# jrcalgo/RelayRL-prototype

Hardware: AMD Instinct MI355X
Metric: env steps/sec (whole node) + wall-clock to return threshold, CartPole REINFORCE (higher is better)
Workload: dtype fp32; 1 GPU; global_batch=2097152, seq_len=64, parallelism=dp1, envs_per_gpu=32768, train_vf_iters=80, hyperparams=reference defaults (gamma .98, lam .97, pi_lr 3e-4, vf_lr 1e-3)

## Files before the change

### csrc/kernels/value_grad.hip

```cpp
#include <type_traits>

#include "api.h"
#include "common.h"
#include "grad_args.h"
#include "heads.h"

namespace rrl {

typedef __bf16 vbf16x8 __attribute__((ext_vector_type(8)));
typedef __bf16 vbf16x4 __attribute__((ext_vector_type(4)));
typedef short vs16x4 __attribute__((ext_vector_type(4)));

constexpr int kVgH = 128;
#ifndef VG_MT2
#define VG_MT2 1
#endif
constexpr int kVgLd = 144;
constexpr int kVgImg = 64 * kVgLd;
constexpr int vg_red_bytes(int NA) { return 8 * 64 * NA * 4; }
constexpr int vg_base_bytes(int DP, int NA) {
  return 6 * kVgImg * 2 + 2 * 64 * DP * 4 + (2 + NA) * 128 * 4 + 32 * 4 + kVgH * kVgLd * 2;
}
constexpr bool vg_red_in_image(int DP, int NA) { return vg_base_bytes(DP, NA) + vg_red_bytes(NA) > 160 * 1024; }
constexpr int vg_lds_bytes(int DP, int NA) {
// ... 161 lines not shown
  const vs16x4 hi = __builtin_amdgcn_ds_read_tr16_b64_v4i16((lds_v4*)(a0 + 4 * kVgLd));
  typedef short vs16x8 __attribute__((ext_vector_type(8)));
  const vs16x8 v = __builtin_shufflevector(lo, hi, 0, 1, 2, 3, 4, 5, 6, 7);
  return __builtin_bit_cast(vbf16x8, v);
}
RRL_DEV Split8 frag_tr(const uint16_t* img, int k0, int col0, int lane) {
  Split8 s;
  s.h = frag_tr1(img, k0, col0, lane);
  s.m = frag_tr1(img + kVgImg, k0, col0, lane);
  s.l = frag_tr1(img + 2 * kVgImg, k0, col0, lane);
  return s;
}

RRL_DEV void store_split(uint16_t* img, int row, int col, const floatx4 v) {
  vbf16x4 h, m, lo;
  split4(v, h, m, lo);
  uint16_t* a = img + img_off(row, col);
  *reinterpret_cast<vbf16x4*>(a) = h;
  *reinterpret_cast<vbf16x4*>(a + kVgImg) = m;
  *reinterpret_cast<vbf16x4*>(a + 2 * kVgImg) = lo;
}

struct Pieces {
  vbf16x4 h, m, l;
};
RRL_DEV void store_pieces(uint16_t* img, int row, int col, const Pieces& pc) {
  uint16_t* a = img + img_off(row, col);
  *reinterpret_cast<vbf16x4*>(a) = pc.h;
  *reinterpret_cast<vbf16x4*>(a + kVgImg) = pc.m;
  *reinterpret_cast<vbf16x4*>(a + 2 * kVgImg) = pc.l;
}

template <int CTRL>
RRL_DEV float dpp_f(float v) {
  return __int_as_float(__builtin_amdgcn_update_dpp(0, __float_as_int(v), CTRL, 0xf, 0xf, true));
}
constexpr int kDppXor8 = 0x128;
constexpr int kDppMirror8 = 0x141;
constexpr int kDppXor2 = 0x4e;
constexpr int kDppXor1 = 0xb1;

RRL_DEV float reduce_scatter16(const float (&v)[16], int j) {
  float u[8], w4[4], w2[2];
#pragma unroll
  for (int k = 0; k < 8; ++k) {
    const bool hi = j & 8;
    const float send = hi ? v[k] : v[k + 8], keep = hi ? v[k + 8] : v[k];
    u[k] = keep + dpp_f<kDppXor8>(send);
  }
#pragma unroll
  for (int k = 0; k < 4; ++k) {
    const bool hi = j & 4;
    const float send = hi ? u[k] : u[k + 4], keep = hi ? u[k + 4] : u[k];
    w4[k] = keep + dpp_f<kDppMirror8>(send);
  }
#pragma unroll
  for (int k = 0; k < 2; ++k) {
    const bool hi = j & 2;
    const float send = hi ? w4[k] : w4[k + 2], keep = hi ? w4[k + 2] : w4[k];
    w2[k] = keep + dpp_f<kDppXor2>(send);
  }
  const bool hi = j & 1;
  const float send = hi ? w2[0] : w2[1], keep = hi ? w2[1] : w2[0];
  return keep + dpp_f<kDppXor1>(send);
}

RRL_DEV float wave_sum_vl(float v) {
  v += dpp_f<kDppXor1>(v);
  v += dpp_f<kDppXor2>(v);
  v += dpp_f<kDppMirror8>(v);
  v += dpp_f<kDppXor8>(v);
  return group_sum_swap(v);
}

#define VG_STAMP(k)                                                                     \
  if (STAMP) {                                                                          \
    __builtin_amdgcn_sched_barrier(0);                                                  \
    unsigned long long t_;                                                              \
    asm volatile("s_memtime %0\n\ts_waitcnt lgkmcnt(0)" : "=s"(t_)::"memory");          \
    __builtin_amdgcn_sched_barrier(0);                                                  \
    if ((k) > 0) st_sum[(k) > 0 ? (k)-1 : 0] += t_ - st_prev;                           \
    st_prev = t_;                                                                       \
  }

constexpr int vg_prod_v(int DP) { return DP <= 4 ? 7 : 1; }

template <int DP, int HEAD, int NA, bool STAMP = false, int V = vg_prod_v(DP), bool FWD = false>
__global__ __launch_bounds__(512, 1) void value_grad_split_kernel(GradArgs p) {
  unsigned long long st_prev = 0, st_sum[12] = {0, 0, 0, 0, 0, 0, 0, 0, 0, 0, 0, 0};
  unsigned long long st_entry = 0;
  if (STAMP) asm volatile("s_memtime %0\n\ts_waitcnt lgkmcnt(0)" : "=s"(st_entry)::"memory");
  extern __shared__ __attribute__((aligned(16))) uint16_t vg_lds[];
  constexpr bool kValue = HEAD == HEAD_VALUE_MSE;
  constexpr bool kGauss = HEAD == HEAD_PG_GAUSS || HEAD == HEAD_PPO_GAUSS;
  constexpr bool kPPO = HEAD == HEAD_PPO_CAT || HEAD == HEAD_PPO_GAUSS;
  static_assert(!kValue || NA == 1, "the value head has one output");
  static_assert(!FWD || kValue, "the forward-only instance is the value head's");
  static_assert(NA >= 1 && NA <= 6, "NA <= 6 (LDS plan, two field groups)");
  static_assert(!vg_split_head(HEAD, NA) || (NA % 2 == 0 && NA <= 6),
                "the dout table is read in output pairs; head MFMA lanes g = 0, 1 hold outputs 0..7");
  constexpr bool kFactor = vg_factor(DP, HEAD, NA) && !FWD;
  constexpr bool kBin = kFactor && !kValue;
  constexpr bool kMaskB = kFactor && (V & 1);
  constexpr bool kInterleave = kMaskB && (V & 2);
  constexpr bool kPipe = kInterleave && !FWD && vg_pipe(DP, HEAD, V);
  constexpr int NF = NA + 2;
  constexpr int NG = (NF + 3) / 4;
  constexpr bool kRedImg = vg_red_in_image(DP, NA);
  constexpr bool kSplitHead = vg_split_head(HEAD, NA);
  uint16_t* h1img = vg_lds;
  uint16_t* dhimg = vg_lds + 3 * kVgImg;
  float* tail = reinterpret_cast<float*>(vg_lds + 6 * kVgImg);
  float* red = kRedImg ? reinterpret_cast<float*>(dhimg) : tail;
  float* xsb = kRedImg ? tail : tail + 8 * NA * 64;
  float* vecs = xsb + 2 * 64 * DP;
  uint16_t* w2lo = reinterpret_cast<uint16_t*>(vecs + (2 + NA) * kVgH + 32);
  uint32_t* mk = reinterpret_cast<uint32_t*>(w2lo + kVgH * kVgLd);
  const vbf16x8* mtab = reinterpret_cast<const vbf16x8*>(mk + 64 * 4);
  float* hbuf0 = kRedImg ? red + 8 * NA * 64
                         : reinterpret_cast<float*>(reinterpret_cast<char*>(mk) + vg_mask_bytes(DP, HEAD, NA));
  float* dtab = reinterpret_cast<float*>(
      reinterpret_cast<char*>(mk) + vg_mask_bytes(DP, HEAD, NA) +
      (kRedImg ? 0 : (vg_hbuf2(DP, HEAD, NA) ? 2 : 1) * vg_hbuf_bytes(HEAD, NA)));
  float* hacc = dtab + 64 * NA;
  float* xs3 = reinterpret_cast<float*>(reinterpret_cast<char*>(vg_lds) + vg_total_bytes(DP, HEAD, NA));
  uint16_t* mbt = reinterpret_cast<uint16_t*>(xs3 + 64 * DP) + 64 * (threadIdx.x >> 6);
  uint16_t* dpt = reinterpret_cast<uint16_t*>(xs3 + 64 * DP) + 8 * 64;
  if (kSplitHead && lane_id() < 2 * NA) hacc[(threadIdx.x >> 6) * 2 * NA + lane_id()] = 0.f;
  if (kMaskB) {
    for (int q = threadIdx.x; q < 256 * 4; q += blockDim.x) {
      const int i = q >> 2, e = 2 * (q & 3);
      mk[64 * 4 + q] = (((i >> e) & 1) ? 0x3F80u : 0u) | (((i >> (e + 1)) & 1) ? 0x3F800000u : 0u);
    }
  }
  int parity = 0;
  int xi = 0;
  constexpr int KS1 = DP / 4;
  const int l = lane_id();
  const int j = l & 15, g = l >> 4, w = threadIdx.x >> 6;
  const int D = p.D;
  const int Bv = p.nvalid ? min(*p.nvalid, p.B) : p.B;
  const int Bc = max(Bv, 1);
  const float invB = p.inv_B_dev ? *p.inv_B_dev : p.inv_B;
  const FlatOffsets o = flat_offsets(D, kVgH, NA);
  float adv_mean = 0.f, adv_rstd = 1.f;
  if (!kValue && p.adv_stats != nullptr) {
    const float n = fmaxf(p.adv_stats[2], 1.f);
    adv_mean = p.adv_stats[0] / n;
    const float var = fmaxf(p.adv_stats[1] / n - adv_mean * adv_mean, 0.f);
    adv_rstd = 1.f / (sqrtf(var) + 1e-8f);
  }
  const float* __restrict__ P = p.params;
  const int own = 16 * w;
  auto frag_slot = [&]() {
    int ll = l;
    asm volatile("" : "+v"(ll));
    return (ll & 32) + 8 * ((ll >> 2) & 3) + ((ll >> 2) & 4) + (ll & 3);
  };

  constexpr int NC = kGauss ? NA : 1;
  const int wu = __builtin_amdgcn_readfirstlane(w);
  auto dma = [&](const void* src, long n, long first, float* dst, int chunks, int w0) {
    for (int k = 0; k < chunks; ++k) {
      if (((k + w0) & 7) == wu) {
        const long e = min(first + 64L * k + l, n - 1);
        __builtin_amdgcn_global_load_lds(static_cast<const uint32_t*>(src) + e,
                                         (__attribute__((address_space(3))) void*)(dst + 64 * k), 4, 0, 0);
      }
    }
  };
  constexpr bool kDmaIn = !kValue;
  constexpr int XQ = (64 * DP + 511) / 512;
  float xr[kDmaIn ? 1 : XQ];
  float hin_r = 0.f;
  auto prefetch_x = [&](int b0, float* dst) {
    if (kDmaIn) {
      for (int k = wu; k < DP; k += 8) {
        const int q = 64 * k + l, row = q / DP, d = q % DP;
        const long e = (long)min(b0 + row, Bc - 1) * D + min(d, D - 1);
        __builtin_amdgcn_global_load_lds(static_cast<const uint32_t*>(static_cast<const void*>(p.X)) + e,
                                         (__attribute__((address_space(3))) void*)(dst + 64 * k), 4, 0, 0);
      }
    } else {
#pragma unroll
      for (int i = 0; i < (kDmaIn ? 1 : XQ); ++i) {
        const int q = min((int)threadIdx.x + 512 * i, 64 * DP - 1);
        const int rl = q / DP, d = q % DP, b = b0 + rl;
        xr[i] = p.X[(size_t)min(b, Bc - 1) * D + min(d, D - 1)];
      }
      if (!FWD) hin_r = p.ret[min(b0 + l, p.B - 1)];
    }
  };
  auto xbuf = [&](int i) { return i < 2 ? xsb + i * 64 * DP : xs3; };
  auto load_x = [&](int b0) {
    int tid = threadIdx.x;
    asm volatile("" : "+v"(tid));
#pragma unroll
    for (int i = 0; i < (kDmaIn ? 1 : XQ); ++i) {
      const int q = min(tid + 512 * i, 64 * DP - 1);
      const int rl = q / DP, d = q % DP, b = b0 + rl;
      xr[i] = p.X[(size_t)min(b, Bc - 1) * D + min(d, D - 1)];
    }
  };
  auto store_x = [&](int b0, float* dst) {
    int tid = threadIdx.x;
    asm volatile("" : "+v"(tid));
#pragma unroll
    for (int i = 0; i < (kDmaIn ? 1 : XQ); ++i) {
      const int q = tid + 512 * i;
      const int rl = q / DP, d = q % DP;
      if (q < 64 * DP) dst[q] = (b0 + rl < Bv && d < D) ? xr[i] : 0.f;
    }
  };
  constexpr bool kHb2 = kDmaIn && vg_hbuf2(DP, HEAD, NA);
  constexpr int HBF = vg_hbuf_bytes(HEAD, NA) / 4;
  auto dma_head = [&](int b0, float* hbuf) {
    if (kDmaIn) {
      dma(p.adv, p.B, b0, hbuf, 1, 3);
      if (p.logp_old) dma(p.logp_old, p.B, b0, hbuf + 64, 1, 4);
      if (kGauss) dma(p.actc, (long)p.B * NA, (long)b0 * NA, hbuf + 128, NA, 5);
      else dma(p.act, p.B, b0, hbuf + 128, 1, 5);
    }
  };
  auto vm_wait0 = []() { __builtin_amdgcn_s_waitcnt(0x0F70); };
  prefetch_x(blockIdx.x * 64, xsb);
  if (kHb2) dma_head(blockIdx.x * 64, hbuf0);

  constexpr int kW2Ld = kVgH + 4;
  static_assert(kVgH * kW2Ld * 4 <= 6 * kVgImg * 2, "staged W2 must fit in the activation images");
  float* w2s = reinterpret_cast<float*>(vg_lds);
  float* hsc = vecs + (2 + NA) * kVgH;
  float w1a[KS1];
#pragma unroll
  for (int s = 0; s < KS1; ++s) {
    const int k = 4 * s + g;
    w1a[s] = (k < D) ? P[o.w1 + (own + j) * D + k] : 0.f;
  }
  {
    const float* gw2 = P + o.w2;
    const bool al16 = (reinterpret_cast<uintptr_t>(gw2) & 15) == 0;
    floatx4 v[kVgH * kVgH / 4 / 512];
#pragma unroll
    for (int it = 0; it < kVgH * kVgH / 4 / 512; ++it) {
      const int q = (int)threadIdx.x + 512 * it;
      if (al16) {
        v[it] = *reinterpret_cast<const floatx4*>(gw2 + 4 * q);
      } else {
#pragma unroll
        for (int e = 0; e < 4; ++e) v[it][e] = gw2[4 * q + e];
      }
    }
    for (int q = threadIdx.x; q < (2 + NA) * kVgH; q += blockDim.x) {
      const int k = q >> 7, f = q & (kVgH - 1);
      vecs[q] = P[(k == 0 ? o.b1 : k == 1 ? o.b2 : o.w3 + (k - 2) * kVgH) + f];
    }
    if (threadIdx.x < NA) {
      const int a = threadIdx.x;
      const float lsa = kGauss ? P[o.log_std + a] : 0.f;
      hsc[a] = P[o.b3 + a];
      hsc[NA + a] = lsa;
      hsc[2 * NA + a] = __expf(-lsa);
    }
#pragma unroll
    for (int it = 0; it < kVgH * kVgH / 4 / 512; ++it) {
      const int q = (int)threadIdx.x + 512 * it;
      *reinterpret_cast<floatx4*>(w2s + (q >> 5) * kW2Ld + 4 * (q & 31)) = v[it];
      vbf16x4 h, m, lo;
      split4(v[it], h, m, lo);
      *reinterpret_cast<vbf16x4*>(w2lo + (q >> 5) * kVgLd + 4 * (q & 31)) = lo;
    }
  }
  if constexpr (kPipe) {
    store_x(blockIdx.x * 64, xsb);
    if ((int)(blockIdx.x + gridDim.x) * 64 < Bv) load_x((blockIdx.x + gridDim.x) * 64);
  }
  __syncthreads();
  Split8HM wA[4], wB[4];
  auto w3f = [&](int k) { return kBin ? vecs[3 * kVgH + k] - vecs[2 * kVgH + k] : vecs[2 * kVgH + k]; };
  vbf16x8 wBl[kFactor ? 4 : 1];
#pragma unroll
  for (int c = 0; c < 4; ++c) {
    const floatx4 a0 = *reinterpret_cast<const floatx4*>(w2s + (own + j) * kW2Ld + 32 * c + 8 * g);
    const floatx4 a1 = *reinterpret_cast<const floatx4*>(w2s + (own + j) * kW2Ld + 32 * c + 8 * g + 4);
    const Split8 sa = split8(a0, a1);
// ... 183 lines not shown
      };
      if (base + (int)gridDim.x * 64 < Bv) fwd_steps(std::true_type{});
      else fwd_steps(std::false_type{});
    } else {
      Split8 cur = frag_row(h1img, j, 8 * g);
      vbf16x8 al = *reinterpret_cast<const vbf16x8*>(w2lo + (own + j) * kVgLd + 8 * g);
#pragma unroll
      for (int it = 0; it < 16; ++it) {
        const int c = it >> 2, bt = it & 3;
        Split8 nxt;
        vbf16x8 aln;
        if (it + 1 < 16) nxt = frag_row(h1img, 16 * ((it + 1) & 3) + j, 32 * ((it + 1) >> 2) + 8 * g);
        if (bt == 3 && it + 1 < 16)
          aln = *reinterpret_cast<const vbf16x8*>(w2lo + (own + j) * kVgLd + 32 * (c + 1) + 8 * g);
        const Split8 a{wA[c].h, wA[c].m, al};
        h2[bt] = mma6(a, cur, h2[bt]);
        __builtin_amdgcn_sched_barrier(0);
        if (it + 1 < 16) cur = nxt;
        if (bt == 3 && it + 1 < 16) al = aln;
      }
    }
#pragma unroll
    for (int bt = 0; bt < 4; ++bt) {
#pragma unroll
      for (int r = 0; r < 4; ++r) h2[bt][r] = relu1(h2[bt][r]);
    }
    if (kMaskB) {
      uint32_t x01 = 0, x23 = 0;
#pragma unroll
      for (int bt = 0; bt < 4; ++bt) {
        uint32_t nib = 0;
#pragma unroll
        for (int r = 0; r < 4; ++r) nib |= (h2[bt][r] > 0.f ? 1u : 0u) << r;
        const uint32_t sh = 4 * g + 16 * (bt & 1);
        if (bt < 2) x01 |= nib << sh;
        else x23 |= nib << sh;
      }
      x01 = group_or_swap(x01);
      x23 = group_or_swap(x23);
      const uint32_t u = ((g < 2 ? x01 : x23) >> (16 * (g & 1))) & 0xffffu;
      uint8_t* mb = reinterpret_cast<uint8_t*>(mk) + (16 * g + j) * 16 + 8 * (w & 1) + (w >> 1);
      mb[0] = (uint8_t)(u & 0xffu);
      mb[4] = (uint8_t)(u >> 8);
      if constexpr (kPipe) mbt[frag_slot()] = (uint16_t)u;
    }

    VG_STAMP(3);
    if constexpr (kSplitHead) {
      floatx4 w3m = zero4();
      if (j < NA) w3m = *reinterpret_cast<const floatx4*>(w3p + j * kVgH);
#pragma unroll
      for (int bt = 0; bt < 4; ++bt) {
        floatx4 c = zero4();
#pragma unroll
        for (int r = 0; r < 4; ++r) c = mfma4(w3m[r], h2[bt][r], c);
        float* dst = red + (w * 64 + 16 * bt + j) * NA + 4 * g;
        if (g == 0) {
          *reinterpret_cast<vf32x2*>(dst) = vf32x2{c[0], c[1]};
          *reinterpret_cast<vf32x2*>(dst + 2) = vf32x2{c[2], c[3]};
        } else if (4 * g < NA) {
          *reinterpret_cast<vf32x2*>(dst) = vf32x2{c[0], c[1]};
        }
      }
    } else {
#pragma unroll
    for (int a = 0; a < NA; ++a) {
      const floatx4 w3a = *reinterpret_cast<const floatx4*>(w3p + a * kVgH);
#pragma unroll
      for (int bt = 0; bt < 4; ++bt) {
        float pv = w3a[0] * h2[bt][0];
        pv = fmaf(w3a[1], h2[bt][1], pv);
        pv = fmaf(w3a[2], h2[bt][2], pv);
        pv = fmaf(w3a[3], h2[bt][3], pv);
        pv = group_sum_swap(pv);
        if (g == bt) red[(w * NA + a) * 64 + 16 * bt + j] = pv;
      }
      if (NA > 2) __builtin_amdgcn_sched_barrier(0);
    }
    }
    VG_STAMP(4);
    if (kDmaIn && !kHb2) vm_wait0();
    __syncthreads();
    VG_STAMP(5);
    if constexpr (FWD) {
      if (w == 0 && base + l < Bv) {
        const float* r = red + l;
        p.vout[base + l] = (((r[0] + r[64]) + (r[128] + r[192])) + ((r[256] + r[320]) + (r[384] + r[448]))) + hsc[0];
      }
      if (base + (int)gridDim.x * 64 < Bv) prefetch_x(base + gridDim.x * 64, xsb + (parity & 1) * 64 * DP);
      continue;
    }
    const bool lead = w == 0;
    float dout[NA];
    float dls_row[kGauss ? NA : 1];
    if constexpr (kSplitHead) {
      const int a8 = l & 7, R = 8 * w + (l >> 3);
      const bool va = a8 < NA;
      const int ac = min(a8, NA - 1);
      const bool ok = base + R < Bv;
      const float* rr = red + R * NA + ac;
      constexpr int S = 64 * NA;
      const float outv = (((rr[0] + rr[S]) + (rr[2 * S] + rr[3 * S])) + ((rr[4 * S] + rr[5 * S]) + (rr[6 * S] + rr[7 * S]))) +
                         hsc[ac];
      const float hin = hbuf[R], hlp = hbuf[64 + R];
      const float lsd = hsc[NA + ac], istd = hsc[2 * NA + ac];
      const float d = (ok ? hbuf[128 + R * NA + ac] : outv) - outv;
      const float z = d * istd;
      float logp = va ? -0.5f * z * z - lsd - kHalfLog2Pi : 0.f;
      float ent = va ? 0.5f + kHalfLog2Pi + lsd : 0.f;
      logp += dpp_f<kDppXor1>(logp);
      ent += dpp_f<kDppXor1>(ent);
      logp += dpp_f<kDppXor2>(logp);
      ent += dpp_f<kDppXor2>(ent);
      logp += dpp_f<kDppMirror8>(logp);
      ent += dpp_f<kDppMirror8>(ent);
      const float adv = ((ok ? hin : 0.f) - adv_mean) * adv_rstd;
      float dlogp, loss_i;
      if (!kPPO) {
        dlogp = -adv;
        loss_i = -logp * adv;
      } else {
        const float lpo = (ok && p.logp_old) ? hlp : logp;
        const float ratio = __expf(logp - lpo);
        const float s1 = ratio * adv;
        const float s2 = fminf(fmaxf(ratio, 1.f - p.clip_eps), 1.f + p.clip_eps) * adv;
        dlogp = (s1 <= s2) ? -adv * ratio : 0.f;
        loss_i = -fminf(s1, s2);
        if (a8 == 0 && ok) s_clip += (fabsf(ratio - 1.f) > p.clip_eps) ? 1.f : 0.f;
      }
      const float scale = (ok && va) ? invB : 0.f;
      const float iv = istd * istd;
      const float da = scale * dlogp * d * iv;
      const float dl = scale * (dlogp * (d * d * iv - 1.f) - p.ent_coef);
      if (va) dtab[R * NA + a8] = da;
      const float hb = group_sum_swap(da + dpp_f<kDppXor8>(da));
      const float hl = group_sum_swap(dl + dpp_f<kDppXor8>(dl));
      if (l < NA) {
        hacc[w * 2 * NA + l] += hb;
        hacc[w * 2 * NA + NA + l] += hl;
      }
      if (a8 == 0 && ok) {
        s_loss += loss_i;
        s_ent += ent;
        if (p.logp_old) s_kl += hlp - logp;
        s_cnt += 1.f;
      }
    } else {
      const int b = base + l;
      const bool ok = b < Bv;
      const int bc = min(b, p.B - 1);
      const float hin = kDmaIn ? hbuf[l] : hin_r;
      const float hlp = kValue ? 0.f : hbuf[64 + l];
      const int hact = (kValue || kGauss) ? 0 : __float_as_int(hbuf[128 + l]);
      float hac[NC];
#pragma unroll
      for (int a = 0; a < NC; ++a) hac[a] = kGauss ? hbuf[128 + l * NC + a] : 0.f;
      float outv[NA];
#pragma unroll
      for (int a = 0; a < NA; ++a) {
        const float* r = red + a * 64 + l;
        constexpr int S = NA * 64;
        outv[a] = (((r[0] + r[S]) + (r[2 * S] + r[3 * S])) + ((r[4 * S] + r[5 * S]) + (r[6 * S] + r[7 * S]))) + hsc[a];
      }
      if (kValue) {
        const float v = outv[0];
        const float diff = v - (ok ? hin : 0.f);
        dout[0] = ok ? 2.f * diff * invB : 0.f;
        if (lead && ok) {
          s_loss += diff * diff;
          s_val += v;
          s_cnt += 1.f;
        }
      } else {
        const float adv = ((ok ? hin : 0.f) - adv_mean) * adv_rstd;
        float logp = 0.f, ent = 0.f;
        float logits[kMaxAct];
        CatStats cs{0.f, 0.f};
        int act = 0;
        if (kGauss) {
#pragma unroll
          for (int a = 0; a < NA; ++a) {
            const float xa = ok ? hac[a % NC] : outv[a];
            const float z = (xa - outv[a]) * hsc[2 * NA + a];
            logp += -0.5f * z * z - hsc[NA + a] - kHalfLog2Pi;
            ent += 0.5f + kHalfLog2Pi + hsc[NA + a];
          }
        } else {
#pragma unroll
          for (int a = 0; a < kMaxAct; ++a) logits[a] = a < NA ? outv[a] : -INFINITY;
          if (ok) apply_mask(p.mask ? p.mask + (size_t)bc * NA : nullptr, NA, logits);
          cs = cat_stats(NA, logits);
          act = ok ? hact : 0;
          logp = pick_logit(NA, logits, act) - cs.lse;
          ent = cs.entropy;
        }
        float dlogp, loss_i;
        if (!kPPO) {
          dlogp = -adv;
          loss_i = -logp * adv;
        } else {
          const float lpo = (ok && p.logp_old) ? hlp : logp;
          const float ratio = __expf(logp - lpo);
          const float s1 = ratio * adv;
          const float s2 = fminf(fmaxf(ratio, 1.f - p.clip_eps), 1.f + p.clip_eps) * adv;
          dlogp = (s1 <= s2) ? -adv * ratio : 0.f;
          loss_i = -fminf(s1, s2);
          if (lead && ok) s_clip += (fabsf(ratio - 1.f) > p.clip_eps) ? 1.f : 0.f;
        }
        const float scale = ok ? invB : 0.f;
#pragma unroll
        for (int a = 0; a < NA; ++a) {
          if (kGauss) {
            const float d = (ok ? hac[a % NC] : outv[a]) - outv[a];
            const float iv = hsc[2 * NA + a] * hsc[2 * NA + a];
            dout[a] = scale * dlogp * d * iv;
            dls_row[a % NC] = scale * (dlogp * (d * d * iv - 1.f) - p.ent_coef);
          } else {
            const float lpa = logits[a] - cs.lse;
            const float pa = __expf(lpa);
            const float dpg = dlogp * ((a == act ? 1.f : 0.f) - pa);
            const float dent = pa > 0.f ? p.ent_coef * pa * (lpa + cs.entropy) : 0.f;
            dout[a] = scale * (dpg + dent);
          }
        }
        if (lead && ok) {
          s_loss += loss_i;
          s_ent += ent;
          if (p.logp_old) s_kl += hlp - logp;
          s_cnt += 1.f;
        }
      }
      float mb = 0.f, ml = 0.f;
#pragma unroll
      for (int a = 0; a < NA; ++a) {
        if (a == w) {
          mb = dout[a];
          if (kGauss) ml = dls_row[a % NC];
        }
      }
      if (w < NA) {
        bacc3 += wave_sum_vl(mb);
        if (kGauss) dls += wave_sum_vl(ml);
      }
    }
    auto prefetch_next = [&]() {
      if (base + (int)gridDim.x * 64 < Bv) {
        prefetch_x(base + gridDim.x * 64, xsb + (parity & 1) * 64 * DP);
        if (kHb2) dma_head(base + gridDim.x * 64, hbuf0 + (parity & 1) * HBF);
      }
    };
    constexpr bool kHeadBar = kRedImg || kSplitHead;
    if constexpr (kPipe) {
      const int stride = (int)gridDim.x * 64;
      if (base + stride < Bv) {
        hin_r = p.ret[min(base + stride + l, p.B - 1)];
        if (base + 2 * stride < Bv) load_x(base + 2 * stride);
      }
    } else if (!kHeadBar && kFactor) {
      prefetch_next();
    }
    if (kHeadBar) {
      __syncthreads();
      prefetch_next();
    }

    VG_STAMP(6);
    floatx4 dh1[4];
#pragma unroll
    for (int bt = 0; bt < 4; ++bt) dh1[bt] = zero4();
    auto dh1_relu = [&]() {
#pragma unroll
      for (int cc = 0; cc < 2; ++cc) {
        typedef unsigned short vu16x8 __attribute__((ext_vector_type(8)));
        const vu16x8 hb = __builtin_bit_cast(vu16x8, frag_tr1(h1s, 32 * cc, own, l));
#pragma unroll
        for (int e = 0; e < 8; ++e) {
          const int bt = 2 * cc + (e >> 2), i = e & 3;
          dh1[bt][i] = hb[e] != 0 ? dh1[bt][i] : 0.f;
          db1acc += dh1[bt][i];
        }
      }
    };
    constexpr bool kDwTab = vg_dw_bytes(DP, HEAD, NA) > 0 && (kMaskB || !kFactor);
    float* dtw = reinterpret_cast<float*>(reinterpret_cast<char*>(vg_lds) + vg_total_bytes(DP, HEAD, NA) -
                                          vg_dw_bytes(DP, HEAD, NA)) + 64 * w;
    if (kFactor) {
      const float dfac = kBin ? 0.5f * (dout[NA - 1] - dout[0]) : dout[0];
      float dv[4];
      if (kMaskB) {
        dtw[l] = dfac;
        __builtin_amdgcn_fence(__ATOMIC_ACQ_REL, "wavefront");
        __builtin_amdgcn_wave_barrier();
#pragma unroll
        for (int bt = 0; bt < 4; ++bt) dv[bt] = dtw[16 * bt + j];
      } else {
#pragma unroll
        for (int bt = 0; bt < 4; ++bt) dv[bt] = __shfl(dfac, 16 * bt + j, 64);
      }
      float* tv = tvs;
      if (!kTvPersist) {
#pragma unroll
        for (int e = 0; e < 16; ++e) tvs[e % (kFactor ? 16 : 1)] = 0.f;
      }
      auto kf_tile = [&](const int bt) {
        const float v = dv[bt];
        if constexpr (!kPipe) {
          uint32_t ph, pm, pl;
          split2(vf32x2{v, v}, ph, pm, pl);
          uint32_t mw[2];
#pragma unroll
          for (int q = 0; q < 2; ++q) {
            const bool p0 = h2[bt][2 * q] > 0.f, p1 = h2[bt][2 * q + 1] > 0.f;
            mw[q] = (p0 ? 0x0000ffffu : 0u) | (p1 ? 0xffff0000u : 0u);
          }
          Pieces pc;
          pc.h = __builtin_bit_cast(vbf16x4, make_uint2(mw[0] & ph, mw[1] & ph));
          pc.m = __builtin_bit_cast(vbf16x4, make_uint2(mw[0] & pm, mw[1] & pm));
          pc.l = __builtin_bit_cast(vbf16x4, make_uint2(mw[0] & pl, mw[1] & pl));
          store_pieces(dhimg, 16 * bt + j, own + 4 * g, pc);
        }
#pragma unroll
        for (int r = 0; r < 4; ++r) {
          tv[r] += h2[bt][r] > 0.f ? v : 0.f;
          tv[4 + r] = fmaf(v, h2[bt][r], tv[4 + r]);
        }
      };
      auto kf_finish = [&]() {
        if (!kTvPersist) accv[0] += fold_tvs();
        if (kMaskB) {
          __builtin_amdgcn_fence(__ATOMIC_ACQ_REL, "wavefront");
          __builtin_amdgcn_wave_barrier();
        }
      };
      auto kf_dh2 = [&]() {
#pragma unroll
        for (int bt = 0; bt < 4; ++bt) kf_tile(bt);
        kf_finish();
      };
      auto kf_dh1 = [&]() {
        if (kMaskB) {
          uint32_t mrow[4];
#pragma unroll
          for (int bt = 0; bt < 4; ++bt) mrow[bt] = mk[(16 * bt + j) * 4 + g];
          constexpr int kAhead = VG_MT2 ? 2 : 1;
          auto mfrag = [&](int it) { return mtab[(mrow[it & 3] >> (8 * (it >> 2))) & 0xffu]; };
          vbf16x8 q0 = mfrag(0), q1;
          if (kAhead == 2) q1 = mfrag(1);
#pragma unroll
          for (int it = 0; it < 16; ++it) {
            const int c = it >> 2, bt = it & 3;
            vbf16x8 nxt;
            if (it + kAhead < 16) nxt = mfrag(it + kAhead);
            dh1[bt] = mfma_bf16(q0, wBl[c % (kFactor ? 4 : 1)], dh1[bt]);
            dh1[bt] = mfma_bf16(q0, wB[c].m, dh1[bt]);
            dh1[bt] = mfma_bf16(q0, wB[c].h, dh1[bt]);
            if constexpr (kPipe) {
              if (it == 0) {
                uint32_t ph, pm, pl;
                split2(vf32x2{dfac, dfac}, ph, pm, pl);
                uint16_t* dp = dpt + frag_slot();
                dp[0] = (uint16_t)ph;
                dp[64] = (uint16_t)pm;
                dp[128] = (uint16_t)pl;
              }
            }
            if (kInterleave) {
              if ((it & 3) == 1) kf_tile(it >> 2);
              if (it == 15) kf_finish();
            }
            if constexpr (kPipe) __builtin_amdgcn_sched_group_barrier(0x100, 1, 0);
            __builtin_amdgcn_sched_barrier(0);
            if (kAhead == 2) {
              q0 = q1;
              if (it + 2 < 16) q1 = nxt;
            } else if (it + 1 < 16) {
              q0 = nxt;
            }
          }
        } else {
          vbf16x8 cur = *reinterpret_cast<const vbf16x8*>(dhimg + img_off(j, 8 * g));
#pragma unroll
          for (int it = 0; it < 16; ++it) {
            const int c = it >> 2, bt = it & 3;
            vbf16x8 nxt;
            if (it + 1 < 16)
              nxt = *reinterpret_cast<const vbf16x8*>(
                  dhimg + img_off(16 * ((it + 1) & 3) + j, 32 * ((it + 1) >> 2) + 8 * g));
            dh1[bt] = mfma_bf16(cur, wBl[c % (kFactor ? 4 : 1)], dh1[bt]);
            dh1[bt] = mfma_bf16(cur, wB[c].m, dh1[bt]);
            dh1[bt] = mfma_bf16(cur, wB[c].h, dh1[bt]);
            __builtin_amdgcn_sched_barrier(0);
            if (it + 1 < 16) cur = nxt;
          }
        }
        float sr = dfac;
        if (!kMaskB) {
          const float vh = __uint_as_float(cvt_pk_bf16(sr, sr) << 16);
          sr = vh != 0.f ? sr * __builtin_amdgcn_rcpf(vh) : 0.f;
        }
        if (kMaskB) {
#pragma unroll
          for (int bt = 0; bt < 4; ++bt) {
            const floatx4 d4 = *reinterpret_cast<const floatx4*>(dtw + 16 * bt + 4 * g);
#pragma unroll
            for (int i = 0; i < 4; ++i) dh1[bt][i] *= d4[i];
          }
        } else {
#pragma unroll
          for (int bt = 0; bt < 4; ++bt) {
#pragma unroll
            for (int i = 0; i < 4; ++i) dh1[bt][i] *= __shfl(sr, 16 * bt + 4 * g + i, 64);
          }
        }
        dh1_relu();
      };
      if (kInterleave) {
        VG_STAMP(7);
        kf_dh1();
      } else {
        kf_dh2();
        if (!kMaskB) __syncthreads();
        VG_STAMP(7);
        kf_dh1();
      }
    } else {
      floatx4 dd[4];
      if constexpr (kSplitHead) {
        const float* w3v = vecs + 2 * kVgH + own + j;
        const float wk0 = g < NA ? w3v[g * kVgH] : 0.f;
        const float wk1 = 4 + g < NA ? w3v[(4 + g) * kVgH] : 0.f;
#pragma unroll
        for (int bt = 0; bt < 4; ++bt) {
          const float* dr = dtab + (16 * bt + j) * NA;
          const float b0 = g < NA ? dr[g] : 0.f;
          const float b1 = 4 + g < NA ? dr[4 + g] : 0.f;
          dd[bt] = mfma4(wk1, b1, mfma4(wk0, b0, zero4()));
        }
      } else {
#pragma unroll
        for (int bt = 0; bt < 4; ++bt) dd[bt] = zero4();
      }
      auto tab_pair = [&](int a2, vf32x2(&q)[4]) {
#pragma unroll
        for (int bt = 0; bt < 4; ++bt) q[bt] = *reinterpret_cast<const vf32x2*>(dtab + (16 * bt + j) * NA + a2);
      };
      vf32x2 vq[4];
      if (kDwTab) {
        dtw[l] = dout[0];
        __builtin_amdgcn_fence(__ATOMIC_ACQ_REL, "wavefront");
        __builtin_amdgcn_wave_barrier();
      }
      {
        float tv[16];
#pragma unroll
        for (int e = 0; e < 16; ++e) tv[e] = 0.f;
#pragma unroll
        for (int a = 0; a < NA; ++a) {
          if (kSplitHead && (a & 1) == 0) tab_pair(a, vq);
          const floatx4 w3a = kSplitHead ? zero4() : *reinterpret_cast<const floatx4*>(w3p + a * kVgH);
          const int f = a == 0 ? 1 : 3;
#pragma unroll
          for (int bt = 0; bt < 4; ++bt) {
            const float v = kSplitHead ? vq[bt][a & 1] : kDwTab ? dtw[16 * bt + j] : __shfl(dout[a], 16 * bt + j, 64);
#pragma unroll
            for (int r = 0; r < 4; ++r) {
              if (!kSplitHead) dd[bt][r] = fmaf(w3a[r], v, dd[bt][r]);
              if (a < 2) tv[4 * f + r] = fmaf(v, h2[bt][r], tv[4 * f + r]);
            }
          }
          if (kSplitHead && (a & 1)) __builtin_amdgcn_sched_barrier(0);
        }
#pragma unroll
        for (int bt = 0; bt < 4; ++bt) {
#pragma unroll
          for (int r = 0; r < 4; ++r) {
            dd[bt][r] = h2[bt][r] > 0.f ? dd[bt][r] : 0.f;
// ... 175 lines not shown
#pragma unroll
      for (int r = 0; r < 4; ++r) slab[o.w2 + (own + 4 * g + r) * kVgH + 16 * it + j] = acc2[it][r] * w3s[r];
    }
#pragma unroll
    for (int q = 0; q < NG; ++q) {
      const int f = 4 * q + (j >> 2), feat = own + 4 * g + (j & 3);
      if (f < NF) {
        const int off = f == 0 ? o.b2 : f == 1 ? o.w3 : f == 2 ? o.b1 : o.w3 + (f == 3 ? 1 : f - 2) * kVgH;
        if (f != 2) slab[off + feat] = (kFactor && f == 0) ? accv[q] * w3g(feat) : accv[q];
      }
    }
    if (kDw1Mfma) {
#pragma unroll
      for (int nt = 0; nt < (kDw1Mfma ? NT1 : 1); ++nt) {
#pragma unroll
        for (int i = 0; i < 4; ++i) {
          const int d = 16 * nt + j;
          if (d < D) slab[o.w1 + (own + 4 * g + i) * D + d] = acc1m[nt][i];
        }
      }
#pragma unroll
      for (int e = 0; e < kTail1; ++e) {
        const float sd = group_sum_swap(acc1[e % NA1]);
        const int d = 16 * NT1 + e;
        if (g == e && d < D) slab[o.w1 + (own + j) * D + d] = sd;
      }
    } else {
#pragma unroll
      for (int d = 0; d < NA1; ++d) {
        const float sd = group_sum_swap(acc1[d]);
        if (g == (d & 3) && d < D) slab[o.w1 + (own + j) * D + d] = sd;
      }
    }
    {
      const float sb = group_sum_swap(db1acc);
      if (g == 0) slab[o.b1 + own + j] = sb;
    }
    if constexpr (kSplitHead) {
      const float st[6] = {wave_sum_vl(s_loss), wave_sum_vl(s_ent), wave_sum_vl(s_kl),
                           wave_sum_vl(s_clip), wave_sum_vl(s_val), wave_sum_vl(s_cnt)};
      __syncthreads();
      float* ep = dtab;
      if (l == 0) {
#pragma unroll
        for (int k = 0; k < 6; ++k) ep[w * 6 + k] = st[k];
      }
      __syncthreads();
      const int t = threadIdx.x;
      if (t < 2 * NA) {
        float v = 0.f;
#pragma unroll
        for (int ww = 0; ww < 8; ++ww) v += hacc[ww * 2 * NA + t];
        slab[(t < NA ? o.b3 : o.log_std - NA) + t] = v;
      } else if (t >= 64 && t < 70) {
        float v = 0.f;
#pragma unroll
        for (int ww = 0; ww < 8; ++ww) v += ep[ww * 6 + t - 64];
        p.loss_slab[blockIdx.x * 8 + t - 64] = v;
      }
    }
    if (!kSplitHead && w < NA && l == 0) {
      slab[o.b3 + w] = bacc3;
      if (kGauss) slab[o.log_std + w] = dls;
    }
    if (!kSplitHead && w == 0) {
      const float sl = wave_sum(s_loss), sv = wave_sum(s_val), sc = wave_sum(s_cnt);
      const float se = wave_sum(s_ent), sk = wave_sum(s_kl), scl = wave_sum(s_clip);
      if (l == 0) {
        float* lsl = p.loss_slab + blockIdx.x * 8;
        lsl[0] = sl;
        lsl[1] = se;
        lsl[2] = sk;
        lsl[3] = scl;
        lsl[4] = sv;
        lsl[5] = sc;
      }
    }
    if (STAMP && p.stamps != nullptr) {
      unsigned long long t_end;
      asm volatile("s_memtime %0\n\ts_waitcnt lgkmcnt(0)" : "=s"(t_end)::"memory");
      st_sum[11] = t_end - st_prev;
      if (l == 0) {
#pragma unroll
        for (int k = 0; k < 12; ++k) p.stamps[(blockIdx.x * 8 + w) * 16 + k] = st_sum[k];
      }
    }
  }
}

bool value_grad_split_supported(int D, int H) { return H == kVgH && D >= 1 && D <= 24; }

bool policy_grad_split_supported(int D, int H, int A, int head) {
  if (H != kVgH || D < 1) return false;
  if (head == HEAD_PG_CAT || head == HEAD_PPO_CAT) return D <= 8 && A >= 2 && A <= 4;
  if (head == HEAD_PG_GAUSS || head == HEAD_PPO_GAUSS) return D <= 20 && (A == 1 || A == 6);
  return false;
}

static int g_vg_tune = 0;
static unsigned long long* g_vg_stamps = nullptr;

template <int DP, int HEAD, int NA, bool STAMP, int V>
static int launch_inst(const GradArgs& a, int grid, hipStream_t s) {
  constexpr int bytes = vg_total_bytes(DP, HEAD, NA) + vg_pipe_bytes(DP, HEAD, V);
  static_assert(bytes <= 160 * 1024, "value-grad LDS plan exceeds 160 KB");
  static bool attr_set = false;
  if (!attr_set) {
    (void)hipFuncSetAttribute((const void*)value_grad_split_kernel<DP, HEAD, NA, STAMP, V>,
                              hipFuncAttributeMaxDynamicSharedMemorySize, bytes);
    attr_set = true;
  }
  hipLaunchKernelGGL((value_grad_split_kernel<DP, HEAD, NA, STAMP, V>), dim3(grid), dim3(512), bytes, s, a);
  return (int)hipGetLastError();
}

template <int DP, int HEAD, int NA, bool STAMP>
static int launch_var(const GradArgs& a, int grid, hipStream_t s) {
  if constexpr (HEAD == HEAD_VALUE_MSE && DP <= 8) {
    if (a.tune & 128) {
      switch ((a.tune >> 4) & 7) {
        case 0: return launch_inst<DP, HEAD, NA, STAMP, 0>(a, grid, s);
        case 1: return launch_inst<DP, HEAD, NA, STAMP, 1>(a, grid, s);
        case 3: return launch_inst<DP, HEAD, NA, STAMP, 3>(a, grid, s);
        case 7:
          if constexpr (DP == 4) return launch_inst<DP, HEAD, NA, STAMP, 7>(a, grid, s);
          break;
        default: break;
      }
    }
  }
  if constexpr (vg_pipe(DP, HEAD, vg_prod_v(DP))) {
    if ((long)a.B <= 64L * grid) return launch_inst<DP, HEAD, NA, STAMP, 3>(a, grid, s);
  }
  return launch_inst<DP, HEAD, NA, STAMP, vg_prod_v(DP)>(a, grid, s);
}

template <int DP, int HEAD, int NA>
static int launch_vg(const GradArgs& a0, int grid, hipStream_t s) {
  GradArgs a = a0;
  a.tune = g_vg_tune;
  a.stamps = g_vg_stamps;
  if (a.tune & 8) return launch_var<DP, HEAD, NA, true>(a, grid, s);
  return launch_var<DP, HEAD, NA, false>(a, grid, s);
}

int launch_value_grad_split(const GradArgs& a, int grid, hipStream_t s) {
  if (a.D <= 4) return launch_vg<4, HEAD_VALUE_MSE, 1>(a, grid, s);
  if (a.D <= 8) return launch_vg<8, HEAD_VALUE_MSE, 1>(a, grid, s);
  if (a.D <= 16) return launch_vg<16, HEAD_VALUE_MSE, 1>(a, grid, s);
  if (a.D <= 20) return launch_vg<20, HEAD_VALUE_MSE, 1>(a, grid, s);
  return launch_vg<24, HEAD_VALUE_MSE, 1>(a, grid, s);
}

template <int DP>
static int launch_fwd(const GradArgs& a0, int grid, hipStream_t s) {
  constexpr int bytes = vg_total_bytes(DP, HEAD_VALUE_MSE, 1);
  static_assert(bytes <= 160 * 1024, "value-forward LDS plan exceeds 160 KB");
  auto* kern = value_grad_split_kernel<DP, HEAD_VALUE_MSE, 1, false, vg_prod_v(DP), true>;
  static bool attr_set = false;
  if (!attr_set) {
    (void)hipFuncSetAttribute((const void*)kern, hipFuncAttributeMaxDynamicSharedMemorySize, bytes);
    attr_set = true;
  }
  GradArgs a = a0;
  a.tune = 0;
  a.stamps = nullptr;
  hipLaunchKernelGGL(kern, dim3(grid), dim3(512), bytes, s, a);
// ... 63 lines not shown
```

Baseline: 33.10 million env_steps/s.

## Fold value-head loss computation into the MFMA dh1 loop in pipelined path

For the pipelined value-gradient variant, the per-row head work (reduction reads, MSE diff, dout, loss accumulation, next-batch prefetch) moves from a separate serial section into the dh1 MFMA loop, interleaved at specific iterations. The kf_tile scheduling is shifted to make room, and a new per-tile finish applies the dout scale and ReLU mask, reading h1 through a transposed LDS read. load_x is rewritten with 24-bit multiplies and byte offsets off a row base to cut address arithmetic, and extra sub-stamps are added for profiling. This aims to hide head latency behind matrix work, at the cost of higher register pressure and tricky ordering.

```diff
diff --git a/csrc/kernels/value_grad.hip b/csrc/kernels/value_grad.hip
--- a/csrc/kernels/value_grad.hip
+++ b/csrc/kernels/value_grad.hip
@@ -267,12 +267,21 @@
     if ((k) > 0) st_sum[(k) > 0 ? (k)-1 : 0] += t_ - st_prev;                           \
     st_prev = t_;                                                                       \
   }
+#define VG_SUBSTAMP(slot)                                                               \
+  if (STAMP) {                                                                          \
+    __builtin_amdgcn_sched_barrier(0);                                                  \
+    unsigned long long t_;                                                              \
+    asm volatile("s_memtime %0\n\ts_waitcnt lgkmcnt(0)" : "=s"(t_)::"memory");          \
+    __builtin_amdgcn_sched_barrier(0);                                                  \
+    st_sum[slot] += t_ - st_sub;                                                        \
+    st_sub = t_;                                                                        \
+  }
 
 constexpr int vg_prod_v(int DP) { return DP <= 4 ? 7 : 1; }
 
 template <int DP, int HEAD, int NA, bool STAMP = false, int V = vg_prod_v(DP), bool FWD = false>
 __global__ __launch_bounds__(512, 1) void value_grad_split_kernel(GradArgs p) {
-  unsigned long long st_prev = 0, st_sum[12] = {0, 0, 0, 0, 0, 0, 0, 0, 0, 0, 0, 0};
+  unsigned long long st_prev = 0, st_sub = 0, st_sum[14] = {0, 0, 0, 0, 0, 0, 0, 0, 0, 0, 0, 0, 0, 0};
   unsigned long long st_entry = 0;
   if (STAMP) asm volatile("s_memtime %0\n\ts_waitcnt lgkmcnt(0)" : "=s"(st_entry)::"memory");
   extern __shared__ __attribute__((aligned(16))) uint16_t vg_lds[];
@@ -380,11 +389,14 @@
   auto load_x = [&](int b0) {
     int tid = threadIdx.x;
     asm volatile("" : "+v"(tid));
+    const char* xrow = reinterpret_cast<const char*>(p.X + (size_t)b0 * D);
+    const int rmax = Bc - 1 - b0;
 #pragma unroll
     for (int i = 0; i < (kDmaIn ? 1 : XQ); ++i) {
-      const int q = min(tid + 512 * i, 64 * DP - 1);
-      const int rl = q / DP, d = q % DP, b = b0 + rl;
-      xr[i] = p.X[(size_t)min(b, Bc - 1) * D + min(d, D - 1)];
+      const unsigned q = (unsigned)min(tid + 512 * i, 64 * DP - 1);
+      const int rl = (int)(q / DP), d = (int)(q % DP);
+      const unsigned off = (__umul24((unsigned)min(rl, rmax), (unsigned)D) + (unsigned)min(d, D - 1)) * 4u;
+      xr[i] = *reinterpret_cast<const float*>(xrow + off);
     }
   };
   auto store_x = [&](int b0, float* dst) {
@@ -734,6 +746,7 @@
     if (kDmaIn && !kHb2) vm_wait0();
     __syncthreads();
     VG_STAMP(5);
+    if (STAMP) st_sub = st_prev;
     if constexpr (FWD) {
       if (w == 0 && base + l < Bv) {
         const float* r = red + l;
@@ -797,7 +810,7 @@
         if (p.logp_old) s_kl += hlp - logp;
         s_cnt += 1.f;
       }
-    } else {
+    } else if constexpr (!kPipe) {
       const int b = base + l;
       const bool ok = b < Bv;
       const int bc = min(b, p.B - 1);
@@ -814,6 +827,7 @@
         constexpr int S = NA * 64;
         outv[a] = (((r[0] + r[S]) + (r[2 * S] + r[3 * S])) + ((r[4 * S] + r[5 * S]) + (r[6 * S] + r[7 * S]))) + hsc[a];
       }
+      VG_SUBSTAMP(12);
       if (kValue) {
         const float v = outv[0];
         const float diff = v - (ok ? hin : 0.f);
@@ -894,6 +908,7 @@
         bacc3 += wave_sum_vl(mb);
         if (kGauss) dls += wave_sum_vl(ml);
       }
+      VG_SUBSTAMP(13);
     }
     auto prefetch_next = [&]() {
       if (base + (int)gridDim.x * 64 < Bv) {
@@ -902,14 +917,8 @@
       }
     };
     constexpr bool kHeadBar = kRedImg || kSplitHead;
-    if constexpr (kPipe) {
-      const int stride = (int)gridDim.x * 64;
-      if (base + stride < Bv) {
-        hin_r = p.ret[min(base + stride + l, p.B - 1)];
-        if (base + 2 * stride < Bv) load_x(base + 2 * stride);
-      }
-    } else if (!kHeadBar && kFactor) {
-      prefetch_next();
+    if constexpr (!kPipe) {
+      if (!kHeadBar && kFactor) prefetch_next();
     }
     if (kHeadBar) {
       __syncthreads();
@@ -936,16 +945,74 @@
     constexpr bool kDwTab = vg_dw_bytes(DP, HEAD, NA) > 0 && (kMaskB || !kFactor);
     float* dtw = reinterpret_cast<float*>(reinterpret_cast<char*>(vg_lds) + vg_total_bytes(DP, HEAD, NA) -
                                           vg_dw_bytes(DP, HEAD, NA)) + 64 * w;
+    auto dh1_tile_finish = [&](const int bt) {
+      typedef __attribute__((address_space(3))) vs16x4 lds_v4;
+      typedef unsigned short vu16x4 __attribute__((ext_vector_type(4)));
+      const floatx4 d4 = *reinterpret_cast<const floatx4*>(dtw + 16 * bt + 4 * g);
+      const uint16_t* a0 = h1s + img_off(16 * bt + 4 * g + ((l >> 2) & 3), own + 4 * (l & 3));
+      const vu16x4 hb = __builtin_bit_cast(vu16x4, __builtin_amdgcn_ds_read_tr16_b64_v4i16((lds_v4*)(a0)));
+#pragma unroll
+      for (int i = 0; i < 4; ++i) dh1[bt][i] *= d4[i];
+#pragma unroll
+      for (int i = 0; i < 4; ++i) {
+        dh1[bt][i] = hb[i] != 0 ? dh1[bt][i] : 0.f;
+        db1acc += dh1[bt][i];
+      }
+    };
     if (kFactor) {
-      const float dfac = kBin ? 0.5f * (dout[NA - 1] - dout[0]) : dout[0];
+      float dfac = kPipe ? 0.f : kBin ? 0.5f * (dout[NA - 1] - dout[0]) : dout[0];
       float dv[4];
-      if (kMaskB) {
+      float hpart[kPipe ? 8 : 1], hb3 = 0.f, hcur = 0.f;
+      auto pipe_head_reads = [&]() {
+        const float* r = red + l;
+#pragma unroll
+        for (int k = 0; k < (kPipe ? 8 : 1); ++k) hpart[k] = r[64 * k];
+        hb3 = hsc[0];
+        hcur = hin_r;
+        const int stride = (int)gridDim.x * 64;
+        if (base + stride < Bv) {
+          const int nb = base + stride;
+          const char* rrow = reinterpret_cast<const char*>(p.ret + nb);
+          hin_r = *reinterpret_cast<const float*>(rrow + 4u * (unsigned)min(l, p.B - 1 - nb));
+          if (base + 2 * stride < Bv) load_x(base + 2 * stride);
+        }
+      };
+      auto pipe_head_dout = [&]() {
+        constexpr int K = kPipe ? 1 : 0;
+        const bool ok = base + l < Bv;
+        const float v = (((hpart[0] + hpart[K]) + (hpart[2 * K] + hpart[3 * K])) +
+                         ((hpart[4 * K] + hpart[5 * K]) + (hpart[6 * K] + hpart[7 * K]))) + hb3;
+        const float diff = v - (ok ? hcur : 0.f);
+        dfac = ok ? 2.f * diff * invB : 0.f;
         dtw[l] = dfac;
         __builtin_amdgcn_fence(__ATOMIC_ACQ_REL, "wavefront");
         __builtin_amdgcn_wave_barrier();
+        if (lead) {
+          if (ok) {
+            s_loss += diff * diff;
+            s_val += v;
+            s_cnt += 1.f;
+          }
+          bacc3 += wave_sum_vl(dfac);
+        }
+      };
+      auto pipe_head_rows = [&]() {
 #pragma unroll
         for (int bt = 0; bt < 4; ++bt) dv[bt] = dtw[16 * bt + j];
-      } else {
+        uint32_t ph, pm, pl;
+        split2(vf32x2{dfac, dfac}, ph, pm, pl);
+        uint16_t* dp = dpt + frag_slot();
+        dp[0] = (uint16_t)ph;
+        dp[64] = (uint16_t)pm;
+        dp[128] = (uint16_t)pl;
+      };
+      if (kMaskB && !kPipe) {
+        dtw[l] = dfac;
+        __builtin_amdgcn_fence(__ATOMIC_ACQ_REL, "wavefront");
+        __builtin_amdgcn_wave_barrier();
+#pragma unroll
+        for (int bt = 0; bt < 4; ++bt) dv[bt] = dtw[16 * bt + j];
+      } else if (!kMaskB) {
 #pragma unroll
         for (int bt = 0; bt < 4; ++bt) dv[bt] = __shfl(dfac, 16 * bt + j, 64);
       }
@@ -994,6 +1061,7 @@
           uint32_t mrow[4];
 #pragma unroll
           for (int bt = 0; bt < 4; ++bt) mrow[bt] = mk[(16 * bt + j) * 4 + g];
+          if constexpr (kPipe) pipe_head_reads();
           constexpr int kAhead = VG_MT2 ? 2 : 1;
           auto mfrag = [&](int it) { return mtab[(mrow[it & 3] >> (8 * (it >> 2))) & 0xffu]; };
           vbf16x8 q0 = mfrag(0), q1;
@@ -1007,16 +1075,11 @@
             dh1[bt] = mfma_bf16(q0, wB[c].m, dh1[bt]);
             dh1[bt] = mfma_bf16(q0, wB[c].h, dh1[bt]);
             if constexpr (kPipe) {
-              if (it == 0) {
-                uint32_t ph, pm, pl;
-                split2(vf32x2{dfac, dfac}, ph, pm, pl);
-                uint16_t* dp = dpt + frag_slot();
-                dp[0] = (uint16_t)ph;
-                dp[64] = (uint16_t)pm;
-                dp[128] = (uint16_t)pl;
-              }
-            }
-            if (kInterleave) {
+              if (it == 0) pipe_head_dout();
+              if (it == 1) pipe_head_rows();
+              if (it >= 4 && it % 3 == 1) kf_tile((it - 4) / 3);
+              if (it == 15) kf_finish();
+            } else if (kInterleave) {
               if ((it & 3) == 1) kf_tile(it >> 2);
               if (it == 15) kf_finish();
             }
@@ -1044,6 +1107,11 @@
             __builtin_amdgcn_sched_barrier(0);
             if (it + 1 < 16) cur = nxt;
           }
+        }
+        if constexpr (kPipe) {
+#pragma unroll
+          for (int bt = 0; bt < 4; ++bt) dh1_tile_finish(bt);
+          return;
         }
         float sr = dfac;
         if (!kMaskB) {
@@ -1385,7 +1453,7 @@
       st_sum[11] = t_end - st_prev;
       if (l == 0) {
 #pragma unroll
-        for (int k = 0; k < 12; ++k) p.stamps[(blockIdx.x * 8 + w) * 16 + k] = st_sum[k];
+        for (int k = 0; k < 14; ++k) p.stamps[(blockIdx.x * 8 + w) * 16 + k] = st_sum[k];
       }
     }
   }
```

Result: no change. 33.35 million env_steps/s, median of 6 (+0.8%).
